# Lemok00/IDEAS

Measured on AMD Instinct MI355X. Metric: train images/sec at 256x256 (G+D+Ex step), higher is better.
Workload: dtype f32; 1 GPU; IDEAS N=1 sigma=1 256x256 batch=32/GPU full G+D+Ex iteration (lazy R1 every 16, EMA), full-width nets, HIP kernels (BASELINE.json configs[2]); global_batch=32, parallelism=dp1, r1_steps_in_window=0, ranks=1

## Files before the change

### ideas_amd/_lib.py

```python
from __future__ import annotations

import ctypes as C
import os
from typing import Optional

import torch

_HERE = os.path.dirname(os.path.abspath(__file__))
LIB_PATH = os.environ.get("IDEAS_HIP_LIB", os.path.join(_HERE, "libideas_hip.so"))

NCHW, NHWC = 0, 1
F32 = 0
F32_B3 = 1
BF16 = 2
F16 = 3
F64 = 4


def act_dtype(t: torch.Tensor) -> int:
    if t.dtype == torch.float32:
        return F32
    if t.dtype == torch.bfloat16:
        return BF16
    raise RuntimeError(f"ideas_amd: only float32 and bfloat16 activations are implemented, got {t.dtype}")
# ... 52 lines not shown
    "ideas_stream_create": (C.c_int, [C.POINTER(C.c_void_p), C.c_int]),
    "ideas_stream_destroy": (C.c_int, [_P]),
    "ideas_fused_bias_act": (C.c_int, [_P, _P, _P, _P, _P, C.c_int64, C.c_int, C.c_int64, C.c_int, C.c_int, C.c_int,
                                       C.c_float, C.c_float, C.c_int, _P]),
    "ideas_upfirdn2d": (C.c_int, [_P, _P, _P] + [C.c_int] * 14 + [C.c_float, C.c_int, C.c_int, C.c_int, _P]),
    "ideas_fir_up2_add": (C.c_int, [_P, _P, _P, _P] + [C.c_int] * 8 + [C.c_float, C.c_int, C.c_int, _P]),
    "ideas_blur_fused": (C.c_int, [_P, _P, _P] + [C.c_int] * 8 + [C.c_float, C.c_int, C.c_int, _P, _P, _P, C.c_float, C.c_float,
                                   C.c_int, _P]),
    "ideas_conv_igemm": (C.c_int, [_P, _P, _P, _P, _P, _P, _P, C.POINTER(ConvParams), C.c_int, _P]),
    "ideas_conv_igemm_multi": (C.c_int, [C.c_int, _P, _P, C.POINTER(C.c_void_p), _P, _P, C.POINTER(ConvParams), C.c_int, _P]),
    "ideas_b3_conv_supported": (C.c_int, [C.POINTER(ConvParams)]),
    "ideas_b3_wgrad_supported": (C.c_int, [C.POINTER(ConvParams)]),
    "ideas_b3_wgrad3_supported": (C.c_int, [C.POINTER(ConvParams)]),
    "ideas_b3_wino_supported": (C.c_int, [C.POINTER(ConvParams)]),
    "ideas_b3_wino_split_weights": (C.c_int, [_P, _P, C.c_int, C.c_int, C.c_int64, C.c_int64, C.c_int64, C.c_int64, C.c_int64, _P]),
    "ideas_b3_split_weights": (C.c_int, [_P, _P, C.c_int, C.c_int, C.c_int, _P]),
    "ideas_b3_split_weights_strided": (C.c_int, [_P, _P] + [C.c_int] * 4 + [C.c_int64] * 4 + [_P]),
    "ideas_bf16_conv_supported": (C.c_int, [C.POINTER(ConvParams), C.c_int]),
    "ideas_bf16_wgrad_supported": (C.c_int, [C.POINTER(ConvParams), C.c_int]),
    "ideas_bf16_direct_supported": (C.c_int, [C.POINTER(ConvParams)]),
    "ideas_bf16_pack_weights": (C.c_int, [_P, _P, _P, C.c_int, C.c_int, C.c_int, C.c_int, _P]),
    "ideas_bf16_pack_weights_strided": (C.c_int, [_P, _P, _P] + [C.c_int] * 5 + [C.c_int64] * 4 + [_P]),
    "ideas_conv3x3_wino": (C.c_int, [_P, _P, _P, _P, _P, _P, _P, C.POINTER(ConvParams), C.c_int, _P]),
    "ideas_conv3x3_wino_wgrad": (C.c_int, [_P, _P, _P, _P, _P, C.POINTER(ConvParams), C.c_int, _P]),
    "ideas_wino_wgrad_fold": (C.c_int, [_P, _P, C.c_int, C.c_int] + [C.c_int64] * 4 + [C.c_int, _P]),
    "ideas_b3_blur_conv_s2_supported": (C.c_int, [C.POINTER(ConvParams), C.c_int, C.c_int, C.c_int]),
    "ideas_b3_blur_conv_s2": (C.c_int, [_P, _P, _P, _P, C.POINTER(C.c_float), C.POINTER(C.c_float), _P, _P, C.POINTER(ConvParams),
                                        C.c_int, C.c_int, C.c_int, _P]),
    "ideas_b3_blur_conv_s2_mod": (C.c_int, [_P, _P, _P, _P, C.POINTER(C.c_float), C.POINTER(C.c_float), _P, _P, _P, _P,
                                            C.POINTER(ConvParams), C.c_int, C.c_int, C.c_int, _P]),
    "ideas_conv_direct": (C.c_int, [_P, _P, _P, _P, _P, _P, _P, C.POINTER(ConvParams), C.c_int, _P]),
    "ideas_conv_wgrad": (C.c_int, [_P, _P, _P, _P, _P, C.POINTER(ConvParams), C.c_int, _P]),
    "ideas_conv_wgrad_direct": (C.c_int, [_P, _P, _P, _P, _P, C.POINTER(ConvParams), C.c_int, _P]),
    "ideas_demod": (C.c_int, [_P, _P, _P, C.c_int, C.c_int, C.c_int, C.c_float, _P]),
    "ideas_weight_sqsum": (C.c_int, [_P, _P] + [C.c_int] * 4 + [C.c_int64] * 4 + [C.c_float, _P]),
    "ideas_weight_sqsum_f64": (C.c_int, [_P, _P] + [C.c_int] * 4 + [C.c_int64] * 4 + [C.c_double, _P]),
    "ideas_demod_bwd": (C.c_int, [_P] * 7 + [C.c_int] * 3 + [C.c_float, _P]),
    "ideas_demod_wgrad": (C.c_int, [_P] * 4 + [C.c_int] * 5 + [C.c_int64] * 8 + [C.c_float, _P]),
    "ideas_pixel_dot": (C.c_int, [_P, _P, _P, C.c_int, C.c_int64, C.c_int, C.c_int, _P]),
    "ideas_reflect_fold": (C.c_int, [_P, _P, C.c_int, C.c_int, C.c_int, C.c_int, C.c_int, C.c_int, _P]),
    "ideas_adam_ema": (C.c_int, [_P, _P, _P, _P, C.c_int64, C.c_float, C.c_float, C.c_float, C.c_float, C.c_float, _P]),
    "ideas_image_u8_to_f32": (C.c_int, [_P, _P, _P, C.c_int, C.c_int, C.c_int, C.c_int, C.c_float, C.c_float, _P]),
    "ideas_channel_sum": (C.c_int, [_P, _P, C.c_int64, C.c_int, C.c_int, C.c_int, _P]),
    "ideas_patch_resize": (C.c_int, [_P, _P, C.POINTER(C.c_int)] + [C.c_int] * 8 + [_P]),
    "ideas_patch_resize_bwd": (C.c_int, [_P, _P, C.POINTER(C.c_int)] + [C.c_int] * 9 + [_P]),
    "ideas_sizeof_prep_desc": (C.c_int, []),
    "ideas_weight_prep_batched": (C.c_int, [_P, C.c_int, C.c_int, C.c_int, _P]),
    "ideas_sizeof_linear_seg": (C.c_int, []),
    "ideas_linear_fwd": (C.c_int, [C.POINTER(LinearSeg), C.c_int, _P, C.c_int, C.c_int, C.c_int, _P]),
    "ideas_linear_bwd_x_workspace": (C.c_int64, [C.c_int, C.c_int, C.c_int]),
    "ideas_linear_bwd_x": (C.c_int, [C.POINTER(LinearSeg), C.c_int, _P, C.c_int, C.c_int, C.c_int, _P, C.c_int64, _P]),
    "ideas_linear_bwd_w": (C.c_int, [C.POINTER(LinearSeg), C.c_int, _P, C.c_int, C.c_int, C.c_int, C.c_int, _P]),
    "ideas_act_bwd_dot": (C.c_int, [_P, _P, _P, _P, _P, _P, _P, C.c_int, C.c_int64, C.c_int, C.c_float, C.c_float, C.c_int, _P]),
    "ideas_mbstd_fwd": (C.c_int, [_P, _P, _P] + [C.c_int] * 6 + [C.c_float, C.c_int, _P]),
    "ideas_mbstd_bwd": (C.c_int, [_P, _P, _P, _P] + [C.c_int] * 6 + [C.c_float, C.c_int, _P]),
    "ideas_mbstd_bwd2": (C.c_int, [_P, _P, _P, _P, _P, _P] + [C.c_int] * 6 + [C.c_float, C.c_int, _P]),
    "ideas_noise_bias_act": (C.c_int, [_P] * 5 + [C.c_int] * 5 + [C.c_float, C.c_float, C.c_int, _P]),
    "ideas_noise_bias_act_bwd": (C.c_int, [_P] * 9 + [C.c_int] * 5 + [C.c_float, C.c_float, C.c_int, _P]),
    "ideas_affine_warp": (C.c_int, [_P, _P, _P] + [C.c_int] * 8 + [_P]),
    "ideas_affine_warp_bwd": (C.c_int, [_P, _P, _P] + [C.c_int] * 9 + [_P]),
    "ideas_color_affine": (C.c_int, [_P, _P, _P] + [C.c_int] * 5 + [_P]),
    "ideas_maxpool2x2_fwd": (C.c_int, [_P, _P] + [C.c_int] * 5 + [_P]),
    "ideas_maxpool2x2_bwd": (C.c_int, [_P, _P, _P] + [C.c_int] * 5 + [_P]),
    "ideas_lpips_layer_fwd": (C.c_int, [_P] * 5 + [C.c_int] * 5 + [_P]),
    "ideas_lpips_layer_bwd": (C.c_int, [_P] * 6 + [C.c_int] * 5 + [_P]),
    "ideas_pool3x3_fwd": (C.c_int, [_P, _P] + [C.c_int] * 6 + [_P]),
    "ideas_global_avg_pool": (C.c_int, [_P, _P] + [C.c_int] * 5 + [_P]),
    "ideas_feature_stats_accum": (C.c_int, [_P, _P, _P, C.c_int, C.c_int, _P]),
    "ideas_bits_to_tensor": (C.c_int, [_P, _P, _P, C.c_int, C.c_int, C.c_int, C.c_float, _P]),
    "ideas_tensor_to_bits": (C.c_int, [_P, _P, _P, _P, C.c_int, C.c_int, C.c_int, C.c_int, _P]),
    "ideas_image_f32_to_u8": (C.c_int, [_P, _P, _P] + [C.c_int] * 6 + [_P]),
}
EXPORTS = tuple(_PROTOS)
ABI_VERSION = 4

_lib: Optional[C.CDLL] = None


def load() -> C.CDLL:
    global _lib
    if _lib is not None:
        return _lib
    if not os.path.exists(LIB_PATH):
        raise RuntimeError(
            f"{LIB_PATH} not found: build the HIP extension first (python -c 'import __graft_entry__ as g; g.build()' "
            "or make -C ideas_amd/csrc).  ideas_amd has no CPU / eager fallback.")
    lib = C.CDLL(LIB_PATH)
    ver = getattr(lib, "ideas_abi_version", None)
    if ver is None or ver() != ABI_VERSION:
        raise RuntimeError(f"libideas_hip.so ABI mismatch: the library reports version {None if ver is None else ver()}, this binding "
                           f"needs {ABI_VERSION} (include/ideas_hip.h); rebuild with make -C ideas_amd/csrc")
    for name, (res, args) in _PROTOS.items():
        fn = getattr(lib, name)
        fn.restype = res
        fn.argtypes = args
    if lib.ideas_sizeof_conv_params() != C.sizeof(ConvParams):
        raise RuntimeError("libideas_hip.so ABI mismatch (version or ideas_conv_params layout)")
    if lib.ideas_sizeof_prep_desc() != C.sizeof(PrepDesc):
        raise RuntimeError("libideas_hip.so ABI mismatch (ideas_prep_desc layout)")
    if lib.ideas_sizeof_linear_seg() != C.sizeof(LinearSeg):
        raise RuntimeError("libideas_hip.so ABI mismatch (ideas_linear_seg layout)")
    _lib = lib
    return lib


def check(rc: int, what: str) -> None:
# ... 25 lines not shown
```

### ideas_amd/csrc/upfirdn2d.hip

```cpp
#include "common.hpp"

namespace {

struct FirParams {
    int B, C, in_h, in_w, out_h, out_w, kh, kw;
    int up_x, up_y, down_x, down_y, pad_x0, pad_y0;
    float gain;
    int flip;
    int seg_rows;
};

#define GENERIC_TAP_LDS 32768
template <bool NHWC, typename T, typename A, typename K>
__global__ __launch_bounds__(256) void upfirdn2d_generic(T* __restrict__ y, const T* __restrict__ x,
                                                         const K* __restrict__ fir, FirParams p, int lds_taps) {
    extern __shared__ double s_taps[];
    A* sk = reinterpret_cast<A*>(s_taps);
    if (lds_taps) {
        for (int t = threadIdx.x; t < p.kh * p.kw; t += blockDim.x) {
            int ky = t / p.kw, kx = t % p.kw;
            int src = p.flip ? (p.kh - 1 - ky) * p.kw + (p.kw - 1 - kx) : t;
            sk[t] = (A)fir[src] * (A)p.gain;
        }
        __syncthreads();
// ... 356 lines not shown
        const float4* xr = xb + (int64_t)(rowok ? iy : 0) * p.in_w * C4;
        float4 v[5];
#pragma unroll
        for (int t = 0; t < 5; ++t) {
            const bool ok = rowok && ((colmask >> t) & 1u);
            const float4 w = xr[(int64_t)(ok ? ix0 + t : 0) * C4];
            v[t] = make_float4(ok ? w.x : 0.f, ok ? w.y : 0.f, ok ? w.z : 0.f, ok ? w.w : 0.f);
        }
        ha = zero; hb = zero;
#pragma unroll
        for (int t = 0; t < 5; ++t) {
            if (t < 4) { ha.x = fmaf(v[t].x, kh[t], ha.x); ha.y = fmaf(v[t].y, kh[t], ha.y); ha.z = fmaf(v[t].z, kh[t], ha.z); ha.w = fmaf(v[t].w, kh[t], ha.w); }
            if (t > 0) { hb.x = fmaf(v[t].x, kh[t - 1], hb.x); hb.y = fmaf(v[t].y, kh[t - 1], hb.y); hb.z = fmaf(v[t].z, kh[t - 1], hb.z); hb.w = fmaf(v[t].w, kh[t - 1], hb.w); }
        }
    };
    auto vsum = [&](const float4& r0, const float4& r1, const float4& r2, const float4& r3) {
        return make_float4(r0.x * kv[0] + r1.x * kv[1] + r2.x * kv[2] + r3.x * kv[3], r0.y * kv[0] + r1.y * kv[1] + r2.y * kv[2] + r3.y * kv[3],
                           r0.z * kv[0] + r1.z * kv[1] + r2.z * kv[2] + r3.z * kv[3], r0.w * kv[0] + r1.w * kv[1] + r2.w * kv[2] + r3.w * kv[3]);
    };
    float4 a0, a1, a2, a3, a4, b0, b1, b2, b3, b4;
    {
        const int iy0 = oy0 - p.pad_y0;
        hrow(iy0 + 0, a0, b0); hrow(iy0 + 1, a1, b1); hrow(iy0 + 2, a2, b2);
    }
    int oy = oy0;
#pragma unroll 1
    for (; oy + 1 < oy1; oy += 2) {
        hrow(oy - p.pad_y0 + 3, a3, b3);
        hrow(oy - p.pad_y0 + 4, a4, b4);
        fin(oy, 0, vsum(a0, a1, a2, a3));
        if (colB) fin(oy, 1, vsum(b0, b1, b2, b3));
        fin(oy + 1, 0, vsum(a1, a2, a3, a4));
        if (colB) fin(oy + 1, 1, vsum(b1, b2, b3, b4));
        a0 = a2; a1 = a3; a2 = a4; b0 = b2; b1 = b3; b2 = b4;
    }
    if (oy < oy1) {
        hrow(oy - p.pad_y0 + 3, a3, b3);
        fin(oy, 0, vsum(a0, a1, a2, a3));
        if (colB) fin(oy, 1, vsum(b0, b1, b2, b3));
    }
    if (EPI == EPI_ACT_BWD) {
        const float part[4] = {bsum.x, bsum.y, bsum.z, bsum.w};
        bgrad_flush(s_bg, ep.bgrad, p.C, active, 4 * c4, part, 4);
    }
}
template <int EPI, typename E>
__global__ __launch_bounds__(256) void blur4_bf16x8_c2(uint4* __restrict__ y, const uint4* __restrict__ x,
                                                       const float* __restrict__ fir, FirParams p, FirEpi ep) {
    __shared__ float sk[16];
    extern __shared__ float s_bg[];
    blur4_c2<VecX8<E>, EPI>(y, x, fir, p, ep, sk, s_bg);
}

template <typename T, int EPI>
__global__ __launch_bounds__(256) void blur4_nhwc(typename T::raw* __restrict__ y, const typename T::raw* __restrict__ x,
                                                  const float* __restrict__ fir, FirParams p, FirEpi ep) {
    typedef typename T::raw raw;
    constexpr int N = T::N;
    __shared__ float sk[16];
    extern __shared__ float s_bg[];
    stage_taps(sk, fir, p);
    const int CV = p.C >> T::SHIFT;
    Tile tl;
    const bool active = decode_tile(tl, p, CV, p.out_w, p.out_h);
    if (EPI != EPI_ACT_BWD && !active) return;
    const int ox = tl.col, oy0 = tl.r0, oy1 = tl.r1;
    const int ix0 = ox - p.pad_x0;
    float k[16];
#pragma unroll
    for (int t = 0; t < 16; ++t) k[t] = sk[t];
    const raw* xb = x + (int64_t)tl.b * p.in_h * p.in_w * CV + tl.cv;
    raw* yb = y + (((int64_t)tl.b * p.out_h) * p.out_w + ox) * CV + tl.cv;
    const raw* rb = reinterpret_cast<const raw*>(ep.ref) + (((int64_t)tl.b * p.out_h) * p.out_w + ox) * CV + tl.cv;
    float bb[N] = {}, bsum[N] = {};
    if (EPI == EPI_BIAS_ACT) {
#pragma unroll
        for (int e = 0; e < N; ++e) bb[e] = ep.bias[N * tl.cv + e];
    }
    const unsigned colmask = col_mask<4>(ix0, p.in_w);
    auto row = [&](int iy, Fv<N> (&dst)[4]) { load_row_f<T, 4>(dst, xb, iy, ix0, colmask, p, CV); };
    auto emit = [&](int oy, const Fv<N> (&r0)[4], const Fv<N> (&r1)[4], const Fv<N> (&r2)[4], const Fv<N> (&r3)[4]) {
        float acc[N] = {};
#pragma unroll
        for (int t = 0; t < 4; ++t) {
            const float k0 = k[t], k1 = k[4 + t], k2 = k[8 + t], k3 = k[12 + t];
#pragma unroll
            for (int e = 0; e < N; ++e) acc[e] += r0[t].v[e] * k0 + r1[t].v[e] * k1 + r2[t].v[e] * k2 + r3[t].v[e] * k3;
        }
        finish<T, EPI>(yb, rb, (int64_t)oy * p.out_w * CV, acc, bb, bsum, ep, active);
    };
    Fv<N> w[4][4], w4[4];
    const int iy0 = oy0 - p.pad_y0;
    row(iy0 + 0, w[0]);
    row(iy0 + 1, w[1]);
    row(iy0 + 2, w[2]);
    int oy = oy0;
    for (; oy + 1 < oy1; oy += 2) {
        row(oy - p.pad_y0 + 3, w[3]);
        row(oy - p.pad_y0 + 4, w4);
        emit(oy, w[0], w[1], w[2], w[3]);
        emit(oy + 1, w[1], w[2], w[3], w4);
#pragma unroll
        for (int t = 0; t < 4; ++t) { w[0][t] = w[2][t]; w[1][t] = w[3][t]; w[2][t] = w4[t]; }
    }
    if (oy < oy1) {
        row(oy - p.pad_y0 + 3, w[3]);
// ... 215 lines not shown
            for (int kx = 0; kx < 4; ++kx) acc += sx[ry + ky][rx + kx] * sk[ky * 4 + kx];
        st1(yp + (int64_t)oy * p.out_w + ox, acc);
    }
}

}

#define FIR_LAUNCH(kernel, total, lds, stream, ...) \
    hipLaunchKernelGGL(kernel, dim3((unsigned)ideas_cdiv((int64_t)(total), 256)), dim3(256), lds, stream, __VA_ARGS__)

template <int EPI>
static int launch_blur4(void* y, const void* x, const float* fir, FirParams p, FirEpi ep, int dtype, hipStream_t stream) {
    p.seg_rows = 16;
    const int segs = (p.out_h + p.seg_rows - 1) / p.seg_rows;
    const int64_t total = (int64_t)p.B * segs * p.out_w * (p.C / 4);
    if (ideas_cdiv(total, 256) > 0x7fffffffLL) return IDEAS_E_SHAPE;
    const size_t lds = EPI == EPI_ACT_BWD ? (size_t)p.C * sizeof(float) : 0;
    const int64_t pairs = (int64_t)p.B * segs * ((p.out_w + 1) / 2);
    if constexpr (EPI == EPI_NONE) {
        if (dtype == IDEAS_F16) {
            FIR_LAUNCH((blur4_bf16x8_c2<EPI, _Float16>), pairs * (p.C / 8), lds, stream, (uint4*)y, (const uint4*)x, fir, p, ep);
            return ideas_launch_status();
        }
    }
    if (dtype == IDEAS_BF16 && p.C % 8 == 0)
        FIR_LAUNCH((blur4_bf16x8_c2<EPI, ideas_bf16>), pairs * (p.C / 8), lds, stream, (uint4*)y, (const uint4*)x, fir, p, ep);
    else if (dtype == IDEAS_BF16)
        FIR_LAUNCH((blur4_nhwc<VecBf16x4, EPI>), total, lds, stream, (ideas_bf16x4*)y, (const ideas_bf16x4*)x, fir, p, ep);
    else
        FIR_LAUNCH(blur4_f32_c2<EPI>, pairs * (p.C / 4), lds, stream, (float4*)y, (const float4*)x, fir, p, ep);
    return ideas_launch_status();
}

static void launch_down2(void* y, const void* x, const float* fir, const FirParams& p, int64_t tiles, int dtype, bool x8, hipStream_t stream) {
    if (x8 && dtype == IDEAS_F16)
        FIR_LAUNCH(fir4_down2_bf16x8<_Float16>, tiles * (p.C / 8), 0, stream, (uint4*)y, (const uint4*)x, fir, p);
    else if (x8)
        FIR_LAUNCH(fir4_down2_bf16x8<ideas_bf16>, tiles * (p.C / 8), 0, stream, (uint4*)y, (const uint4*)x, fir, p);
    else if (dtype == IDEAS_BF16)
        FIR_LAUNCH(fir4_down2_nhwc<VecBf16x4>, tiles * (p.C / 4), 0, stream, (ideas_bf16x4*)y, (const ideas_bf16x4*)x, fir, p);
    else
        FIR_LAUNCH(fir4_down2_nhwc<VecF32>, tiles * (p.C / 4), 0, stream, (float4*)y, (const float4*)x, fir, p);
}
static void launch_up2(void* y, const void* x, const float* fir, const FirParams& p, const void* resid, int64_t tiles, int dtype, bool x8,
                       hipStream_t stream) {
    if (x8 && dtype == IDEAS_F16)
        FIR_LAUNCH(fir4_up2<VecX8<_Float16>>, tiles * (p.C / 8), 0, stream, (uint4*)y, (const uint4*)x, fir, p, (const uint4*)resid);
    else if (x8)
        FIR_LAUNCH(fir4_up2<VecX8<ideas_bf16>>, tiles * (p.C / 8), 0, stream, (uint4*)y, (const uint4*)x, fir, p, (const uint4*)resid);
    else if (dtype == IDEAS_BF16)
        FIR_LAUNCH(fir4_up2<VecBf16x4>, tiles * (p.C / 4), 0, stream, (ideas_bf16x4*)y, (const ideas_bf16x4*)x, fir, p, (const ideas_bf16x4*)resid);
    else
        FIR_LAUNCH(fir4_up2<VecF32>, tiles * (p.C / 4), 0, stream, (float4*)y, (const float4*)x, fir, p, (const float4*)resid);
}

#undef FIR_LAUNCH

extern "C" int ideas_blur_fused(void* y, const void* x, const float* fir, int B, int C, int in_h, int in_w, int out_h, int out_w,
                                int pad_x0, int pad_y0, float gain, int flip, int mode, const void* ref, const float* bias,
                                float* bias_grad, float alpha, float scale, int dtype, void* stream_) {
    if (dtype != IDEAS_F32 && dtype != IDEAS_BF16) return IDEAS_E_UNSUPPORTED;
    if (!y || !x || !fir) return IDEAS_E_NULL;
    if (B <= 0 || C <= 0 || in_h <= 0 || in_w <= 0 || out_h <= 0 || out_w <= 0) return IDEAS_E_SHAPE;
    if (C % 4 || C > 8192) return IDEAS_E_UNSUPPORTED;
    if (!ideas_aligned16(x) || !ideas_aligned16(y)) return IDEAS_E_ALIGN;
    FirParams p{B, C, in_h, in_w, out_h, out_w, 4, 4, 1, 1, 1, 1, pad_x0, pad_y0, gain, flip, 16};
    FirEpi ep{ref, bias, bias_grad, alpha, scale};
    hipStream_t stream = (hipStream_t)stream_;
    if (mode == EPI_ACT_BWD) {
        if (!ref || !bias_grad) return IDEAS_E_NULL;
        if (!ideas_aligned16(ref)) return IDEAS_E_ALIGN;
        return launch_blur4<EPI_ACT_BWD>(y, x, fir, p, ep, dtype, stream);
    }
    if (mode == EPI_BIAS_ACT) {
        if (!bias) return IDEAS_E_NULL;
        if (!ideas_aligned16(bias)) return IDEAS_E_ALIGN;
        return launch_blur4<EPI_BIAS_ACT>(y, x, fir, p, ep, dtype, stream);
    }
    return IDEAS_E_UNSUPPORTED;
}

static int upfirdn2d_impl(void* y, const void* x, const float* fir, int B, int C, int in_h, int in_w, int out_h,
                          int out_w, int kh, int kw, int up_x, int up_y, int down_x, int down_y, int pad_x0,
                          int pad_y0, float gain, int flip, int layout, int dtype, void* stream_, const void* resid) {
    if (dtype != IDEAS_F32 && dtype != IDEAS_BF16 && dtype != IDEAS_F16 && dtype != IDEAS_F64) return IDEAS_E_UNSUPPORTED;
    if (dtype == IDEAS_BF16 && layout != IDEAS_NHWC) return IDEAS_E_UNSUPPORTED;
    if (!y || !x || !fir) return IDEAS_E_NULL;
    if (B <= 0 || C <= 0 || in_h <= 0 || in_w <= 0 || out_h <= 0 || out_w <= 0) return IDEAS_E_SHAPE;
    if (kh <= 0 || kw <= 0) return IDEAS_E_UNSUPPORTED;
    if (up_x <= 0 || up_y <= 0 || down_x <= 0 || down_y <= 0) return IDEAS_E_SHAPE;
    if (layout != IDEAS_NCHW && layout != IDEAS_NHWC) return IDEAS_E_UNSUPPORTED;
    hipStream_t stream = (hipStream_t)stream_;
    FirParams p{B, C, in_h, in_w, out_h, out_w, kh, kw, up_x, up_y, down_x, down_y, pad_x0, pad_y0, gain, flip, 16};
    const bool unit = up_x == 1 && up_y == 1 && down_x == 1 && down_y == 1;
    const bool fast = dtype == IDEAS_F32 || dtype == IDEAS_BF16 || (dtype == IDEAS_F16 && C % 8 == 0);
    const bool vec4 = fast && layout == IDEAS_NHWC && kh == 4 && kw == 4 && (C % 4 == 0) && ideas_aligned16(x) && ideas_aligned16(y);
    const bool x8 = (dtype == IDEAS_BF16 || dtype == IDEAS_F16) && C % 8 == 0;
    if (unit && vec4) {
        return launch_blur4<EPI_NONE>(y, x, fir, p, FirEpi{nullptr, nullptr, nullptr, 0.f, 1.f}, dtype, stream);
    }
    if (vec4 && up_x == 1 && up_y == 1 && down_x == 2 && down_y == 2) {
        p.seg_rows = out_h >= 64 ? 16 : 8;
        const int segs = (out_h + p.seg_rows - 1) / p.seg_rows;
        const int64_t tiles = (int64_t)B * segs * out_w;
        if (ideas_cdiv(tiles * (C / 4), 256) > 0x7fffffffLL) return IDEAS_E_SHAPE;
        launch_down2(y, x, fir, p, tiles, dtype, x8, stream);
// ... 68 lines not shown
```

### ideas_amd/op/modulated_conv.py

```python
from __future__ import annotations

import math
from typing import Optional

import torch
from torch.autograd import Function
from torch.autograd.function import once_differentiable

from .. import _lib
from ..precision import to_act, to_f32
from . import conv as _conv
from .conv import conv2d, conv_dgrad_raw, conv_fwd_raw, conv_transpose2d, conv_wgrad_raw, _nhwc
from .conv_plan import ConvGeom, convT_out_size
from . import conv_plan
from . import scratch
from .upfirdn2d import _geometry, blur_bias_act, upfirdn2d, upfirdn2d_raw
from .fused_act import bias_sink, fused_leaky_relu
from .grad_sink import weight_grad


def pixel_dot(a: torch.Tensor, g: torch.Tensor) -> torch.Tensor:
    a, g = _nhwc(a), _nhwc(g)
    b, c, h, w = a.shape
    out = scratch.zeros((b, c), a.device, torch.float64)
    if a.dtype != g.dtype:
        a, g = a.float(), g.float()
    if a.dtype == torch.bfloat16 and c % 4:
        a, g = a.float(), g.float()
    rc = _lib.load().ideas_pixel_dot(_lib.ptr(out), _lib.ptr(a), _lib.ptr(g), b, h * w, c, _lib.act_dtype(a), _lib.stream_ptr())
    _lib.check(rc, "ideas_pixel_dot")
    return out


def weight_sqsum(w: torch.Tensor, scale: float) -> torch.Tensor:
    def make():
        cout, cin, kh, kw = w.shape
        wsq = torch.empty((cout, cin), device=w.device, dtype=torch.float32)
        so, si, sky, skx = w.stride()
        _lib.check(_lib.load().ideas_weight_sqsum(_lib.ptr(wsq), _lib.ptr(w), cout, cin, kh, kw, so, si, sky, skx, float(scale * scale),
                                                  _lib.stream_ptr()), "ideas_weight_sqsum")
        return wsq
    return conv_plan.cached(w, ("wsq", float(scale)), make)


def weight_sqsum_f64(w: torch.Tensor, scale: float) -> torch.Tensor:
    def make():
        cout, cin, kh, kw = w.shape
        wsq = torch.empty((cout, cin), device=w.device, dtype=torch.float64)
        so, si, sky, skx = w.stride()
        _lib.check(_lib.load().ideas_weight_sqsum_f64(_lib.ptr(wsq), _lib.ptr(w), cout, cin, kh, kw, so, si, sky, skx, float(scale * scale),
                                                      _lib.stream_ptr()), "ideas_weight_sqsum_f64")
        return wsq
    return conv_plan.cached(w, ("wsq64", float(scale)), make)


def demod_raw(s: torch.Tensor, wsq: torch.Tensor, eps: float) -> torch.Tensor:
    return _demod_raw(s.detach(), wsq, eps)


def demod_of(w: torch.Tensor, s: torch.Tensor, gain: float, eps: float) -> torch.Tensor:
    sd = s.detach()
    return conv_plan.cached_on(w, ("demod", float(gain), float(eps)), sd, lambda: _demod_raw(sd, weight_sqsum(w, gain), eps))


def _demod_raw(s: torch.Tensor, wsq: torch.Tensor, eps: float) -> torch.Tensor:
    b, cin = s.shape
    cout = wsq.shape[0]
    d = torch.empty((b, cout), device=s.device, dtype=torch.float32)
    rc = _lib.load().ideas_demod(_lib.ptr(d), _lib.ptr(s), _lib.ptr(wsq), b, cin, cout, float(eps), _lib.stream_ptr())
# ... 80 lines not shown


def act_bwd_dot(gy: torch.Tensor, out: torch.Tensor, bias: torch.Tensor, alpha: float, act_gain: float, bias_grad_into=None):
    gy, out = _nhwc(gy), _nhwc(out)
    if gy.dtype != out.dtype:
        gy = gy.to(out.dtype)
    b, c, h, w = out.shape
    gpre = torch.empty_like(out)
    bg = bias_grad_into if bias_grad_into is not None else torch.zeros(c, device=out.device, dtype=torch.float32)
    dot = scratch.zeros((b, c), out.device, torch.float64)
    rc = _lib.load().ideas_act_bwd_dot(_lib.ptr(gpre), _lib.ptr(bg), _lib.ptr(dot), _lib.ptr(gy), _lib.ptr(out),
                                       _lib.ptr(bias), None, b, h * w, c, float(alpha), float(act_gain), _lib.act_dtype(out),
                                       _lib.stream_ptr())
    _lib.check(rc, "ideas_act_bwd_dot")
    return gpre, (None if bias_grad_into is not None else bg), dot


class _ModConvAct(Function):

    @staticmethod
    def forward(ctx, x, w, s, b, gain: float, slope: float, act_gain: float, eps: float):
        x = _nhwc(x)
        bias_param = b
        s, b = s.contiguous(), b.contiguous()
        d = demod_of(w, s, gain, eps)
        k = w.shape[2]
        g = ConvGeom(k, k, 1, k // 2, False)
        y = conv_fwd_raw(x, w, g, gain, lin=s, lout=d, bias=b, act=True, act_gain=act_gain, alpha=slope)
        ctx.g, ctx.gain, ctx.slope, ctx.act_gain, ctx.eps = g, gain, slope, act_gain, eps
        ctx.bias_ref = bias_param
        ctx.save_for_backward(x, w, s, d, b, y)
        return y

    @staticmethod
    @once_differentiable
    def backward(ctx, gy):
        x, w, s, d, b, y = ctx.saved_tensors
        g, gain = ctx.g, ctx.gain
        need_x, need_w, need_s, need_b = ctx.needs_input_grad[:4]
        gpre, gb, dot_d = act_bwd_dot(gy, y, b, ctx.slope, ctx.act_gain, bias_grad_into=bias_sink(ctx.bias_ref) if need_b else None)
        gx = gw = gs = gq = None
        if need_x or need_s:
            gx = conv_dgrad_raw(gpre, w, g, (x.shape[2], x.shape[3]), gain, lin=d, lout=s)
        if need_s or need_w:
            dot_s = pixel_dot(x, gx) if need_s else scratch.zeros(tuple(s.shape), s.device, torch.float64)
            gs, gq = _style_grads(dot_s, dot_d, s, d, w, gain, ctx.eps)
        if need_w:
            def grad(out):
                r = conv_wgrad_raw(gpre, x, g, tuple(w.shape), gain, lin=s, lout=d, out=out)
                _demod_wgrad(r, w, gq, s, gain)
                return r
            gw = weight_grad(w, grad, gpre, x, s, d, gq)
        return (gx if need_x else None), gw, (gs if need_s else None), (gb if need_b else None), None, None, None, None


class _ModConvDown(Function):

    @staticmethod
    def forward(ctx, x, w, s, b, fir, pad2, gain: float, demod: bool, eps: float, slope: float, act_gain: float):
        x = _nhwc(x)
        bias_param = b
        s = s.contiguous()
        act = b is not None
        if act:
            b = b.contiguous()
        d = demod_of(w, s, gain, eps) if demod else None
        k = w.shape[2]
        need_w = ctx.needs_input_grad[1]
        down = 2 if k == 1 else 1
        pad4, bhw, g_pad = _geometry((x.shape[2], x.shape[3]), fir, 1, down, pad2)
        g = ConvGeom(k, k, 1 if k == 1 else 2, 0, False)
        if k == 3 and _conv.mod_blur_conv_ok(x, w, fir, pad2, want_xb=need_w):
            y, xb = _conv.blur_conv_s2_raw(x, w, fir, pad2, gain, bias=b, act=act, act_gain=act_gain, alpha=slope, want_xb=need_w,
                                           lin=s, lout=d)
        else:
            xb = upfirdn2d_raw(x, fir, (1, 1), (down, down), pad4, bhw, flip=True)
            y = conv_fwd_raw(xb, w, g, gain, lin=s, lout=d, bias=b, act=act, act_gain=act_gain, alpha=slope)
        ctx.g, ctx.gain, ctx.has_d, ctx.eps, ctx.act, ctx.slope, ctx.act_gain = g, gain, d is not None, eps, act, slope, act_gain
        ctx.down, ctx.bhw, ctx.g_pad = down, bhw, g_pad
        ctx.bias_ref = bias_param
        none = s.new_zeros(0)
        keep_y = act or d is not None
        ctx.save_for_backward(x, w, s, d if d is not None else none, y if keep_y else none, xb if need_w else none,
                              b if act else none, fir)
        return y

    @staticmethod
    @once_differentiable
    def backward(ctx, gy):
        x, w, s, d, y, xb, b, fir = ctx.saved_tensors
        d = d if ctx.has_d else None
        g, gain = ctx.g, ctx.gain
        need_x, need_w, need_s, need_b = ctx.needs_input_grad[:4]
        gb = dot_d = None
        if ctx.act:
            gpre, gb, dot_d = act_bwd_dot(gy, y, b, ctx.slope, ctx.act_gain, bias_grad_into=bias_sink(ctx.bias_ref) if need_b else None)
        else:
            gpre = gy = _nhwc(gy)
        gx = gw = gs = gq = None
        if need_x or need_s:
            gxb = conv_dgrad_raw(gpre, w, g, ctx.bhw, gain, lin=d, lout=s)
            gx = upfirdn2d_raw(gxb, fir, (ctx.down, ctx.down), (1, 1), ctx.g_pad, (x.shape[2], x.shape[3]), flip=False)
        if need_s or (need_w and d is not None):
            dot_s = pixel_dot(x, gx) if need_s else scratch.zeros(tuple(s.shape), s.device, torch.float64)
            if d is not None and dot_d is None:
                dot_d = pixel_dot(gy, y)
# ... 38 lines not shown
        y = conv_transpose2d(xs, w.transpose(0, 1), None, stride=2, gain=scale)
    else:
        y = conv2d(xs, w, None, stride=1, padding=k // 2, gain=scale)
    if demodulate:
        wsq = (w * w).sum(dim=(2, 3)) * (scale * scale)
        d = torch.rsqrt((style * style) @ wsq.t() + eps)
        y = y * d.view(d.shape[0], cout, 1, 1)
    if upsample:
        p = (fir.shape[0] - 2) - (k - 1)
        y = upfirdn2d(y, fir, pad=((p + 1) // 2 + 1, p // 2 + 1))
    if act_bias is not None:
        y = fused_leaky_relu(y, act_bias, negative_slope, act_scale)
    return y


def modulated_conv2d(x: torch.Tensor, weight: torch.Tensor, style: torch.Tensor, demodulate: bool = True,
                     upsample: bool = False, fir: Optional[torch.Tensor] = None, eps: float = 1e-8,
                     act_bias: Optional[torch.Tensor] = None, negative_slope: float = 0.2,
                     act_scale: float = 2 ** 0.5, resid: Optional[torch.Tensor] = None, downsample: bool = False) -> torch.Tensor:
    if upsample and downsample:
        raise ValueError("modulated_conv2d: upsample and downsample are exclusive")
    _lib.require_cuda(x, weight, style)
    if downsample:
        if fir is None:
            raise RuntimeError("modulated_conv2d(downsample=True) needs the blur FIR")
        if resid is not None:
            raise RuntimeError("modulated_conv2d(resid=...) is the no-grad fast path of the fused same-resolution conv")
        _lib.require_cuda(fir, act_bias)
    x, style = to_act(x), to_f32(style)
    if resid is not None:
        resid = to_act(resid)
    w = weight[0] if weight.dim() == 5 else weight
    cout, cin, k, _ = w.shape
    if _SECOND_ORDER[0] and torch.is_grad_enabled() and resid is None:
        return _modulated_conv2d_composite(x, w, style, demodulate, upsample, fir, eps, act_bias, negative_slope, act_scale, downsample)
    scale = 1.0 / math.sqrt(cin * k * k)
    if downsample:
        fuse = act_bias is not None and demodulate and cout % 4 == 0
        y = _ModConvDown.apply(x, w, style, act_bias if fuse else None, fir, _down_pad(fir, k), scale, bool(demodulate), float(eps),
                               float(negative_slope), float(act_scale))
        return y if (fuse or act_bias is None) else fused_leaky_relu(y, act_bias, negative_slope, act_scale)
    fuse_act = act_bias is not None and not upsample and demodulate and cout % 4 == 0
    if resid is not None:
        if not fuse_act or torch.is_grad_enabled():
            raise RuntimeError("modulated_conv2d(resid=...) is the no-grad fast path of the fused same-resolution conv")
        k_ = w.shape[2]
        style = style.contiguous()
        d = demod_raw(style, weight_sqsum(w, scale), eps)
        return conv_fwd_raw(x, w, ConvGeom(k_, k_, 1, k_ // 2, False), scale, lin=style, lout=d,
                            bias=act_bias.contiguous(), act=True, act_gain=float(act_scale), alpha=float(negative_slope),
                            resid=resid, resid_gain=1.0)
    if fuse_act:
        return _ModConvAct.apply(x, w, style, act_bias, scale, float(negative_slope), float(act_scale), float(eps))
    y = _ModConv.apply(x, w, style, upsample, scale, bool(demodulate), float(eps))
    if upsample:
        if fir is None:
            raise RuntimeError("modulated_conv2d(upsample=True) needs the blur FIR")
        p = (fir.shape[0] - 2) - (k - 1)
        if act_bias is not None:
            return blur_bias_act(y, fir, ((p + 1) // 2 + 1, p // 2 + 1), act_bias, negative_slope, act_scale)
        y = upfirdn2d(y, fir, pad=((p + 1) // 2 + 1, p // 2 + 1))
    if act_bias is not None:
        y = fused_leaky_relu(y, act_bias, negative_slope, act_scale)
    return y
```

### include/ideas_hip.h

```cpp
#ifndef IDEAS_HIP_H
#define IDEAS_HIP_H

#include <stdint.h>

#ifdef __cplusplus
extern "C" {
#endif

#define IDEAS_ABI_VERSION 4

enum { IDEAS_NCHW = 0, IDEAS_NHWC = 1 };
enum { IDEAS_F32 = 0, IDEAS_F32_B3 = 1, IDEAS_BF16 = 2, IDEAS_F16 = 3, IDEAS_F64 = 4 };

enum {
    IDEAS_OK = 0,
    IDEAS_E_NULL = -1,
    IDEAS_E_SHAPE = -2,
    IDEAS_E_UNSUPPORTED = -3,
    IDEAS_E_ALIGN = -4
};

int ideas_abi_version(void);
int ideas_sizeof_conv_params(void);
const char* ideas_strerror(int code);
// ... 60 lines not shown
    const float* w;
    int64_t s[5];
    int a[4];
    int unit;
    int block0;
    int nblocks;
    int pad_;
} ideas_prep_desc;
int ideas_sizeof_prep_desc(void);
int ideas_weight_prep_batched(const ideas_prep_desc* table, int n, int op, int total_blocks, void* stream);
int ideas_bf16_direct_supported(const ideas_conv_params* p);

int ideas_conv_wgrad(float* gw, const void* gy, const void* x, const float* in_scale, const float* out_scale,
                     const ideas_conv_params* p, int dtype, void* stream);

int ideas_conv3x3_wino(void* y, const void* x, const void* umat, const float* in_scale, const float* out_scale,
                       const float* bias, const void* resid, const ideas_conv_params* p, int dtype, void* stream);

int ideas_conv3x3_wino_wgrad(float* gu, const void* gy, const void* x, const float* in_scale, const float* out_scale,
                             const ideas_conv_params* p, int dtype, void* stream);
int ideas_wino_wgrad_fold(float* gw, float* gu, int Cout, int Cin, int64_t so, int64_t sky, int64_t skx, int64_t sc, int clear,
                          void* stream);

int ideas_conv_igemm_multi(int n, void* y, const void* x, const void* const* wmat, const float* in_scale, const float* out_scale,
                           const ideas_conv_params* params, int dtype, void* stream);

int ideas_b3_blur_conv_s2_supported(const ideas_conv_params* p, int xh, int xw, int pad0);
int ideas_b3_blur_conv_s2(void* y, void* xb_out, const void* x, const void* wplanes, const float* fir_h, const float* fir_v,
                          const float* bias, const void* resid, const ideas_conv_params* p, int xh, int xw, int pad0, void* stream);
int ideas_b3_blur_conv_s2_mod(void* y, void* xb_out, const void* x, const void* wplanes, const float* fir_h, const float* fir_v,
                              const float* in_scale, const float* out_scale, const float* bias, const void* resid,
                              const ideas_conv_params* p, int xh, int xw, int pad0, void* stream);

int ideas_conv_direct(void* y, const void* x, const void* wmat, const float* in_scale, const float* out_scale,
                      const float* bias, const void* resid, const ideas_conv_params* p, int dtype, void* stream);
int ideas_conv_wgrad_direct(float* gw, const void* gy, const void* x, const float* in_scale, const float* out_scale,
                            const ideas_conv_params* p, int dtype, void* stream);

int ideas_demod(float* d, const float* s, const float* wsq, int B, int Cin, int Cout, float eps, void* stream);
int ideas_weight_sqsum(float* wsq, const float* w, int Cout, int Cin, int KH, int KW, int64_t so, int64_t si, int64_t sky, int64_t skx,
                       float scale2, void* stream);
int ideas_weight_sqsum_f64(double* wsq, const float* w, int Cout, int Cin, int KH, int KW, int64_t so, int64_t si, int64_t sky,
                           int64_t skx, double scale2, void* stream);
int ideas_demod_bwd(float* gs, float* gq, const double* dot_s, double* dot_d, const float* d, const float* s, const double* wsq,
                    int B, int Cin, int Cout, float eps, void* stream);
int ideas_demod_wgrad(float* gw, const float* w, const float* gq, const float* s, int B, int Cout, int Cin, int KH, int KW, int64_t so,
                      int64_t si, int64_t sky, int64_t skx, int64_t go, int64_t gi, int64_t gky, int64_t gkx, float coef, void* stream);

int ideas_pixel_dot(double* out, const void* a, const void* g, int B, int64_t P, int C, int dtype, void* stream);

int ideas_act_bwd_dot(void* gpre, float* bias_grad, double* dot, const void* gy, const void* out, const float* bias,
                      const float* gpre_scale, int B, int64_t P, int C, float alpha, float act_gain, int dtype, void* stream);

#define IDEAS_MBSTD_MAX_PARTIALS 64
int ideas_mbstd_fwd(void* out, void* workspace, const void* x, int B, int C, int H, int W, int group, int feat, float eps, int dtype,
                    void* stream);
int ideas_mbstd_bwd(void* gx, float* a_out, const void* gout, const void* x, int B, int C, int H, int W, int group, int feat, float eps,
                    int dtype, void* stream);
int ideas_mbstd_bwd2(void* dgout, void* dx, void* workspace, const void* ggx, const void* x, const float* a_in, int B, int C, int H,
                     int W, int group, int feat, float eps, int dtype, void* stream);

#define IDEAS_NOISE_ACT_MAX_PARTIALS 2048
int ideas_noise_bias_act(void* out, const void* x, const float* noise, const float* noise_weight, const float* bias, int B, int C,
                         int H, int W, int noise_batch, float slope, float scale, int dtype, void* stream);
int ideas_noise_bias_act_bwd(void* gx, float* gbias, float* gnw, float* gnoise, void* workspace, const void* gy, const void* out,
                             const float* noise, const float* noise_weight, int B, int C, int H, int W, int noise_batch, float slope,
                             float scale, int dtype, void* stream);

int ideas_reflect_fold(void* gx, const void* gpadded, int B, int H, int W, int C, int pad, int dtype, void* stream);

int ideas_adam_ema(float* p, const float* g, float* v, float* ema, int64_t n, float lr, float beta2, float eps,
                   float bias_correction2, float ema_decay, void* stream);

int ideas_image_u8_to_f32(float* y, const void* x_u8, const void* flip_u8, int B, int H, int W, int C, float mean, float stdv,
                          void* stream);

int ideas_patch_resize(void* y, const void* x, const int* boxes, int n_crop, int B, int C, int H, int W, int out_h, int out_w,
                       int dtype, void* stream);
int ideas_patch_resize_bwd(float* gx, const void* gy, const int* boxes, int n_crop, int B, int C, int H, int W, int out_h,
                           int out_w, int clear, int dtype, void* stream);

int ideas_affine_warp(void* y, const void* x, const float* theta, int B, int C, int H, int W, int OH, int OW, int layout, int dtype,
                      void* stream);
int ideas_affine_warp_bwd(float* gx, const void* gy, const float* theta, int B, int C, int H, int W, int OH, int OW, int clear,
                          int layout, int dtype, void* stream);
int ideas_color_affine(void* y, const void* x, const float* m, int B, int H, int W, int layout, int dtype, void* stream);

#define IDEAS_LPIPS_MAX_PARTIALS 64
int ideas_maxpool2x2_fwd(void* y, const void* x, int B, int C, int H, int W, int dtype, void* stream);
int ideas_maxpool2x2_bwd(void* gx, const void* gy, const void* x, int B, int C, int H, int W, int dtype, void* stream);
int ideas_lpips_layer_fwd(float* d, void* workspace, const void* f0, const void* f1, const float* w, int B, int C, int H, int W,
                          int dtype, void* stream);
int ideas_lpips_layer_bwd(void* gf0, void* gf1, const float* gd, const void* f0, const void* f1, const float* w, int B, int C, int H,
                          int W, int dtype, void* stream);

#define IDEAS_POOL_MAX_S2 0
#define IDEAS_POOL_MAX_S1P1 1
#define IDEAS_POOL_AVG_S1P1_VALID 2
#define IDEAS_FEATURE_STATS_MAX_DIM 4096
int ideas_pool3x3_fwd(void* y, const void* x, int B, int C, int H, int W, int mode, int dtype, void* stream);
int ideas_global_avg_pool(float* out, const void* x, int B, int C, int H, int W, int dtype, void* stream);
int ideas_feature_stats_accum(double* sum, double* gram, const float* x, int N, int D, void* stream);

int ideas_bits_to_tensor(float* z, const void* bits, const float* jitter, int B, int L, int sigma, float delta, void* stream);
int ideas_tensor_to_bits(void* bits, int* n_err, const void* z, const void* ref_bits, int B, int L, int sigma, int dtype,
                         void* stream);
// ... 25 lines not shown
```

Baseline: 84.53 images/sec.

## Fuse upsampling modconv blur+bias+act forward and fused act-backward through blur

Adds a dedicated autograd path for upsampling modulated convs with bias and leaky ReLU. The forward runs the transposed conv, then a single blur kernel with fused bias and activation. The backward uses a new HIP kernel that applies the activation mask, the transposed 4x4 blur, the bias-grad reduction and the demod dot-product accumulation in one pass. This avoids materialising intermediate activation-gradient tensors and extra launches. It adds f64 atomics and shape restrictions: f32 only, padding of 2, and C divisible by 4.

```diff
diff --git a/ideas_amd/_lib.py b/ideas_amd/_lib.py
--- a/ideas_amd/_lib.py
+++ b/ideas_amd/_lib.py
@@ -128,6 +128,7 @@
     "ideas_linear_bwd_x": (C.c_int, [C.POINTER(LinearSeg), C.c_int, _P, C.c_int, C.c_int, C.c_int, _P, C.c_int64, _P]),
     "ideas_linear_bwd_w": (C.c_int, [C.POINTER(LinearSeg), C.c_int, _P, C.c_int, C.c_int, C.c_int, C.c_int, _P]),
     "ideas_act_bwd_dot": (C.c_int, [_P, _P, _P, _P, _P, _P, _P, C.c_int, C.c_int64, C.c_int, C.c_float, C.c_float, C.c_int, _P]),
+    "ideas_act_bwd_blur": (C.c_int, [_P] * 7 + [C.c_int] * 8 + [C.c_float, C.c_int, C.c_float, C.c_float, C.c_int, _P]),
     "ideas_mbstd_fwd": (C.c_int, [_P, _P, _P] + [C.c_int] * 6 + [C.c_float, C.c_int, _P]),
     "ideas_mbstd_bwd": (C.c_int, [_P, _P, _P, _P] + [C.c_int] * 6 + [C.c_float, C.c_int, _P]),
     "ideas_mbstd_bwd2": (C.c_int, [_P, _P, _P, _P, _P, _P] + [C.c_int] * 6 + [C.c_float, C.c_int, _P]),
diff --git a/ideas_amd/csrc/upfirdn2d.hip b/ideas_amd/csrc/upfirdn2d.hip
--- a/ideas_amd/csrc/upfirdn2d.hip
+++ b/ideas_amd/csrc/upfirdn2d.hip
@@ -432,6 +432,162 @@
     blur4_c2<VecX8<E>, EPI>(y, x, fir, p, ep, sk, s_bg);
 }
 
+template <int NCOL>
+__global__ __launch_bounds__(256) void act_bwd_blur4_f32(float4* __restrict__ gx, const float4* __restrict__ gy, const float4* __restrict__ out,
+                                                         const float* __restrict__ fir, FirParams p, FirEpi ep, double* __restrict__ dot) {
+    constexpr int NL = NCOL + 3;
+    __shared__ float sk[16];
+    extern __shared__ double s_dot[];
+    float* s_bg = reinterpret_cast<float*>(s_dot + p.C);
+    stage_taps(sk, fir, p);
+    float kh[4], kv[4];
+    const bool sep = factor_taps(sk, kh, kv);
+    const int C4 = p.C >> 2;
+    const int cols = (p.out_w + NCOL - 1) / NCOL;
+    Tile tl;
+    const bool active = decode_tile(tl, p, C4, cols, p.out_h);
+    const int c4 = tl.cv, b = tl.b, oy0 = tl.r0, oy1 = tl.r1;
+    const int ox = NCOL * tl.col;
+    const int ix0 = ox - p.pad_x0;
+    const float4 zero = make_float4(0.f, 0.f, 0.f, 0.f);
+    const float4* gb = gy + (int64_t)b * p.in_h * p.in_w * C4 + c4;
+    const float4* ob = out + (int64_t)b * p.in_h * p.in_w * C4 + c4;
+    float4* yb = gx + (((int64_t)b * p.out_h) * p.out_w + ox) * C4 + c4;
+    const bool sums = ep.bgrad || dot;
+    const float4 bv = ep.bias ? *reinterpret_cast<const float4*>(ep.bias + 4 * c4) : zero;
+    const float inv_gain = 1.0f / ep.scale, inv_alpha = 1.0f / ep.alpha;
+    float4 bsum = zero;
+    struct { double x, y, z, w; } dsum = {0.0, 0.0, 0.0, 0.0};
+    auto masked = [&](const float4& g, const float4& o) {
+        return make_float4(epi_act(g.x, o.x, ep.alpha, ep.scale), epi_act(g.y, o.y, ep.alpha, ep.scale),
+                           epi_act(g.z, o.z, ep.alpha, ep.scale), epi_act(g.w, o.w, ep.alpha, ep.scale));
+    };
+    auto count = [&](const float4& m, const float4& o) {
+        bsum.x += m.x; bsum.y += m.y; bsum.z += m.z; bsum.w += m.w;
+#define ONE(f)                                                          \
+    {                                                                   \
+        const float t = o.f * inv_gain;                                 \
+        const float pre = ((t > 0.f) ? t : t * inv_alpha) - bv.f;       \
+        dsum.f = fma((double)m.f, (double)pre, dsum.f);                 \
+    }
+        ONE(x) ONE(y) ONE(z) ONE(w)
+#undef ONE
+    };
+    auto store = [&](int oy, int c, const float4& v) {
+        if (active && gx && ox + c < p.out_w) yb[(int64_t)oy * p.out_w * C4 + (int64_t)c * C4] = v;
+    };
+    const unsigned colmask = col_mask<NL>(ix0, p.in_w);
+    if (!sep) {
+#pragma unroll 1
+        for (int oy = oy0; oy < oy1; ++oy)
+#pragma unroll 1
+            for (int c = 0; c < NCOL; ++c) {
+                if (ox + c >= p.out_w) break;
+                float4 acc = zero;
+#pragma unroll 1
+                for (int j = 0; j < 4; ++j) {
+                    const int iy = oy - p.pad_y0 + j;
+                    if (iy < 0 || iy >= p.in_h) continue;
+#pragma unroll 1
+                    for (int t = 0; t < 4; ++t) {
+                        const int ix = ix0 + c + t;
+                        if (ix < 0 || ix >= p.in_w) continue;
+                        const int64_t off = ((int64_t)iy * p.in_w + ix) * C4;
+                        const float4 v = masked(gb[off], ob[off]);
+                        const float kk = sk[4 * j + t];
+                        acc.x = fmaf(v.x, kk, acc.x); acc.y = fmaf(v.y, kk, acc.y); acc.z = fmaf(v.z, kk, acc.z); acc.w = fmaf(v.w, kk, acc.w);
+                    }
+                }
+                store(oy, c, acc);
+                if (sums && active && oy < p.in_h && ox + c < p.in_w) {
+                    const int64_t off = ((int64_t)oy * p.in_w + ox + c) * C4;
+                    const float4 o = ob[off];
+                    count(masked(gb[off], o), o);
+                }
+            }
+    } else {
+        auto hrow = [&](int iy, float4 (&h)[NCOL]) {
+            const bool rowok = (iy >= 0) && (iy < p.in_h);
+            const int64_t roff = (int64_t)(rowok ? iy : 0) * p.in_w * C4;
+            float4 g[NL], o[NL];
+#pragma unroll
+            for (int t = 0; t < NL; ++t) {
+                const bool ok = rowok && ((colmask >> t) & 1u);
+                const int64_t off = roff + (int64_t)(ok ? ix0 + t : 0) * C4;
+                g[t] = gb[off];
+                o[t] = ob[off];
+            }
+#pragma unroll
+            for (int t = 0; t < NL; ++t) {
+                const bool ok = rowok && ((colmask >> t) & 1u);
+                const float4 m = masked(g[t], o[t]);
+                g[t] = make_float4(ok ? m.x : 0.f, ok ? m.y : 0.f, ok ? m.z : 0.f, ok ? m.w : 0.f);
+            }
+#pragma unroll
+            for (int c = 0; c < NCOL; ++c) {
+                h[c] = zero;
+#pragma unroll
+                for (int t = 0; t < 4; ++t) {
+                    h[c].x = fmaf(g[c + t].x, kh[t], h[c].x); h[c].y = fmaf(g[c + t].y, kh[t], h[c].y);
+                    h[c].z = fmaf(g[c + t].z, kh[t], h[c].z); h[c].w = fmaf(g[c + t].w, kh[t], h[c].w);
+                }
+            }
+            if (sums && active && rowok && iy >= oy0 && iy < oy1) {
+#pragma unroll
+                for (int c = 0; c < NCOL; ++c)
+                    if ((colmask >> (2 + c)) & 1u) count(g[2 + c], o[2 + c]);
+            }
+        };
+        auto vsum = [&](const float4& r0, const float4& r1, const float4& r2, const float4& r3) {
+            return make_float4(dot4(r0.x, r1.x, r2.x, r3.x, kv[0], kv[1], kv[2], kv[3]), dot4(r0.y, r1.y, r2.y, r3.y, kv[0], kv[1], kv[2], kv[3]),
+                               dot4(r0.z, r1.z, r2.z, r3.z, kv[0], kv[1], kv[2], kv[3]), dot4(r0.w, r1.w, r2.w, r3.w, kv[0], kv[1], kv[2], kv[3]));
+        };
+        float4 w0[NCOL], w1[NCOL], w2[NCOL], w3[NCOL], w4[NCOL];
+        {
+            const int iy0 = oy0 - p.pad_y0;
+            hrow(iy0 + 0, w0); hrow(iy0 + 1, w1); hrow(iy0 + 2, w2);
+        }
+        int oy = oy0;
+#pragma unroll 1
+        for (; oy + 1 < oy1; oy += 2) {
+            hrow(oy - p.pad_y0 + 3, w3);
+            hrow(oy - p.pad_y0 + 4, w4);
+#pragma unroll
+            for (int c = 0; c < NCOL; ++c) {
+                store(oy, c, vsum(w0[c], w1[c], w2[c], w3[c]));
+                store(oy + 1, c, vsum(w1[c], w2[c], w3[c], w4[c]));
+                w0[c] = w2[c]; w1[c] = w3[c]; w2[c] = w4[c];
+            }
+        }
+        if (oy < oy1) {
+            hrow(oy - p.pad_y0 + 3, w3);
+#pragma unroll
+            for (int c = 0; c < NCOL; ++c) store(oy, c, vsum(w0[c], w1[c], w2[c], w3[c]));
+        }
+    }
+    if (ep.bgrad) {
+        const float part[4] = {bsum.x, bsum.y, bsum.z, bsum.w};
+        bgrad_flush(s_bg, ep.bgrad, p.C, active, 4 * c4, part, 4);
+    }
+    if (dot) {
+        const int segs = (p.out_h + p.seg_rows - 1) / p.seg_rows;
+        const int64_t per_b = (int64_t)segs * cols * C4;
+        const int64_t first = (int64_t)blockIdx.x * blockDim.x;
+        const int b_blk = (int)((first < p.B * per_b ? first : p.B * per_b - 1) / per_b);
+        for (int c = threadIdx.x; c < p.C; c += blockDim.x) s_dot[c] = 0.0;
+        __syncthreads();
+        if (active) {
+            double* dst = (b == b_blk) ? s_dot + 4 * c4 : dot + (int64_t)b * p.C + 4 * c4;
+            atomicAdd(dst + 0, dsum.x); atomicAdd(dst + 1, dsum.y); atomicAdd(dst + 2, dsum.z); atomicAdd(dst + 3, dsum.w);
+        }
+        __syncthreads();
+        for (int c = threadIdx.x; c < p.C; c += blockDim.x) {
+            const double v = s_dot[c];
+            if (v != 0.0) atomicAdd(&dot[(int64_t)b_blk * p.C + c], v);
+        }
+    }
+}
+
 template <typename T, int EPI>
 __global__ __launch_bounds__(256) void blur4_nhwc(typename T::raw* __restrict__ y, const typename T::raw* __restrict__ x,
                                                   const float* __restrict__ fir, FirParams p, FirEpi ep) {
@@ -753,6 +909,31 @@
         FIR_LAUNCH(fir4_up2<VecBf16x4>, tiles * (p.C / 4), 0, stream, (ideas_bf16x4*)y, (const ideas_bf16x4*)x, fir, p, (const ideas_bf16x4*)resid);
     else
         FIR_LAUNCH(fir4_up2<VecF32>, tiles * (p.C / 4), 0, stream, (float4*)y, (const float4*)x, fir, p, (const float4*)resid);
+}
+
+#ifndef IDEAS_ACT_BWD_BLUR_COLS
+#define IDEAS_ACT_BWD_BLUR_COLS 2
+#endif
+
+extern "C" int ideas_act_bwd_blur(void* gx, float* bias_grad, double* dot, const void* gy, const void* out, const float* bias,
+                                  const float* fir, int B, int C, int in_h, int in_w, int out_h, int out_w, int pad_x0, int pad_y0,
+                                  float gain, int flip, float alpha, float scale, int dtype, void* stream_) {
+    if (dtype != IDEAS_F32) return IDEAS_E_UNSUPPORTED;
+    if (!gy || !out || !fir || (!gx && !bias_grad && !dot)) return IDEAS_E_NULL;
+    if (B <= 0 || C <= 0 || in_h <= 0 || in_w <= 0 || out_h <= 0 || out_w <= 0 || C > 3072 || B > 65535) return IDEAS_E_SHAPE;
+    if (out_h < in_h || out_w < in_w) return IDEAS_E_SHAPE;
+    if (pad_x0 != 2 || pad_y0 != 2) return IDEAS_E_UNSUPPORTED;
+    if (C & 3) return IDEAS_E_ALIGN;
+    if (!ideas_aligned16(gy) || !ideas_aligned16(out) || (gx && !ideas_aligned16(gx)) || (bias && !ideas_aligned16(bias))) return IDEAS_E_ALIGN;
+    constexpr int NCOL = IDEAS_ACT_BWD_BLUR_COLS;
+    FirParams p{B, C, in_h, in_w, out_h, out_w, 4, 4, 1, 1, 1, 1, pad_x0, pad_y0, gain, flip, 16};
+    FirEpi ep{nullptr, bias, bias_grad, alpha, scale};
+    const int segs = (out_h + p.seg_rows - 1) / p.seg_rows;
+    const int64_t total = (int64_t)B * segs * ((out_w + NCOL - 1) / NCOL) * (C / 4);
+    if (ideas_cdiv(total, 256) > 0x7fffffffLL) return IDEAS_E_SHAPE;
+    FIR_LAUNCH(act_bwd_blur4_f32<NCOL>, total, (size_t)C * (sizeof(double) + sizeof(float)), (hipStream_t)stream_, (float4*)gx,
+               (const float4*)gy, (const float4*)out, fir, p, ep, dot);
+    return ideas_launch_status();
 }
 
 #undef FIR_LAUNCH
diff --git a/ideas_amd/op/modulated_conv.py b/ideas_amd/op/modulated_conv.py
--- a/ideas_amd/op/modulated_conv.py
+++ b/ideas_amd/op/modulated_conv.py
@@ -1,6 +1,7 @@
 from __future__ import annotations
 
 import math
+import os
 from typing import Optional
 
 import torch
@@ -14,7 +15,7 @@
 from .conv_plan import ConvGeom, convT_out_size
 from . import conv_plan
 from . import scratch
-from .upfirdn2d import _geometry, blur_bias_act, upfirdn2d, upfirdn2d_raw
+from .upfirdn2d import BLUR_BIAS_ACT, _geometry, blur_bias_act, blur_fused_raw, blur_geometry, upfirdn2d, upfirdn2d_raw
 from .fused_act import bias_sink, fused_leaky_relu
 from .grad_sink import weight_grad
 
@@ -201,6 +202,81 @@
                 return r
             gw = weight_grad(w, grad, gpre, x, s, d, gq)
         return (gx if need_x else None), gw, (gs if need_s else None), (gb if need_b else None), None, None, None, None
+
+
+def act_bwd_blur(gy: torch.Tensor, out: torch.Tensor, bias: torch.Tensor, fir: torch.Tensor, g_pad, in_hw, alpha: float, act_gain: float,
+                 want_gx: bool = True, want_dot: bool = True, bias_grad_into=None, want_bias_grad: bool = False):
+    gy, out = _nhwc(gy), _nhwc(out)
+    b, c, h, w = out.shape
+    gx = torch.empty((b, c, in_hw[0], in_hw[1]), device=out.device, dtype=out.dtype, memory_format=torch.channels_last) if want_gx else None
+    bg = bias_grad_into
+    if bg is None and want_bias_grad:
+        bg = torch.zeros(c, device=out.device, dtype=torch.float32)
+    dot = scratch.zeros((b, c), out.device, torch.float64) if want_dot else None
+    if gx is None and bg is None and dot is None:
+        return None, None, None
+    rc = _lib.load().ideas_act_bwd_blur(_lib.ptr(gx), _lib.ptr(bg), _lib.ptr(dot), _lib.ptr(gy), _lib.ptr(out), _lib.ptr(bias), _lib.ptr(fir),
+                                        b, c, h, w, in_hw[0], in_hw[1], g_pad[0], g_pad[2], 1.0, 0, float(alpha), float(act_gain),
+                                        _lib.act_dtype(out), _lib.stream_ptr())
+    _lib.check(rc, "ideas_act_bwd_blur")
+    return gx, (None if bias_grad_into is not None else bg), dot
+
+
+UP_ACT_FUSED = os.environ.get("IDEAS_UP_ACT_FUSED", "1") != "0"
+
+
+def up_act_fused_ok(x: torch.Tensor, w: torch.Tensor, fir: Optional[torch.Tensor]) -> bool:
+    return (UP_ACT_FUSED and fir is not None and tuple(fir.shape) == (4, 4) and w.shape[2] == 3 and x.dim() == 4 and x.is_cuda
+            and x.dtype == torch.float32 and w.shape[0] % 4 == 0 and w.shape[0] <= 3072)
+
+
+class _ModConvUpAct(Function):
+
+    @staticmethod
+    def forward(ctx, x, w, s, b, fir, gain: float, slope: float, act_gain: float, eps: float):
+        x = _nhwc(x)
+        bias_param = b
+        s, b = s.contiguous(), b.contiguous().to(torch.float32)
+        fir = fir.contiguous().to(torch.float32)
+        d = demod_of(w, s, gain, eps)
+        k = w.shape[2]
+        g = ConvGeom(k, k, 2, 0, False)
+        y = conv_dgrad_raw(x, w.transpose(0, 1), g, convT_out_size(x.shape[2], x.shape[3], g), gain, lin=s, lout=d)
+        p = (fir.shape[0] - 2) - (k - 1)
+        pad4, out_hw, g_pad = blur_geometry((y.shape[2], y.shape[3]), fir, ((p + 1) // 2 + 1, p // 2 + 1))
+        out = blur_fused_raw(y, fir, pad4, out_hw, True, BLUR_BIAS_ACT, bias=b, alpha=slope, scale=act_gain)
+        ctx.g, ctx.gain, ctx.slope, ctx.act_gain, ctx.eps = g, gain, slope, act_gain, eps
+        ctx.g_pad, ctx.y_hw = g_pad, (y.shape[2], y.shape[3])
+        ctx.bias_ref = bias_param
+        ctx.save_for_backward(x, w, s, d, b, out, fir)
+        return out
+
+    @staticmethod
+    @once_differentiable
+    def backward(ctx, gy):
+        x, w, s, d, b, out, fir = ctx.saved_tensors
+        g, gain = ctx.g, ctx.gain
+        need_x, need_w, need_s, need_b = ctx.needs_input_grad[:4]
+        need_conv = need_x or need_s or need_w
+        tgt = bias_sink(ctx.bias_ref) if need_b else None
+        gy257, gb, dot_d = act_bwd_blur(gy, out, b, fir, ctx.g_pad, ctx.y_hw, ctx.slope, ctx.act_gain, want_gx=need_conv,
+                                        want_dot=need_s or need_w, bias_grad_into=tgt, want_bias_grad=need_b)
+        gx = gw = gs = gq = None
+        if need_x or need_s:
+            gx = conv_fwd_raw(gy257, w.transpose(0, 1), g, gain, lin=d, lout=s)
+        if need_s or need_w:
+            dot_s = pixel_dot(x, gx) if need_s else scratch.zeros(tuple(s.shape), s.device, torch.float64)
+            gs, gq = _style_grads(dot_s, dot_d, s, d, w, gain, ctx.eps)
+        if need_w:
+            wt_shape = (w.shape[1], w.shape[0], w.shape[2], w.shape[3])
+
+            def grad(o):
+                r = conv_wgrad_raw(x, gy257, g, wt_shape, gain, lin=d, lout=s, out=None if o is None else o.transpose(0, 1)).transpose(0, 1)
+                _demod_wgrad(r, w, gq, s, gain)
+                return r
+            gw = weight_grad(w, grad, x, gy257, s, d, gq)
+        return ((gx if need_x else None), gw, (gs if need_s else None), (gb if (need_b and tgt is None) else None),
+                None, None, None, None, None)
 
 
 class _ModConvDown(Function):
@@ -345,6 +421,8 @@
                             resid=resid, resid_gain=1.0)
     if fuse_act:
         return _ModConvAct.apply(x, w, style, act_bias, scale, float(negative_slope), float(act_scale), float(eps))
+    if upsample and act_bias is not None and demodulate and up_act_fused_ok(x, w, fir):
+        return _ModConvUpAct.apply(x, w, style, act_bias, fir, scale, float(negative_slope), float(act_scale), float(eps))
     y = _ModConv.apply(x, w, style, upsample, scale, bool(demodulate), float(eps))
     if upsample:
         if fir is None:
diff --git a/include/ideas_hip.h b/include/ideas_hip.h
--- a/include/ideas_hip.h
+++ b/include/ideas_hip.h
@@ -136,6 +136,10 @@
 int ideas_act_bwd_dot(void* gpre, float* bias_grad, double* dot, const void* gy, const void* out, const float* bias,
                       const float* gpre_scale, int B, int64_t P, int C, float alpha, float act_gain, int dtype, void* stream);
 
+int ideas_act_bwd_blur(void* gx, float* bias_grad, double* dot, const void* gy, const void* out, const float* bias,
+                       const float* fir, int B, int C, int in_h, int in_w, int out_h, int out_w, int pad_x0, int pad_y0,
+                       float gain, int flip, float alpha, float scale, int dtype, void* stream);
+
 #define IDEAS_MBSTD_MAX_PARTIALS 64
 int ideas_mbstd_fwd(void* out, void* workspace, const void* x, int B, int C, int H, int W, int group, int feat, float eps, int dtype,
                     void* stream);
```

Measured after the change: 85.15 images/sec, median of 6. Within noise of the previous version (+0.7%).
